# SunBangjie/FYP-BidirectionalPathTracer

Hardware: AMD Instinct MI355X
Metric: Mrays/s + RMSE vs the scalar oracle, BDPT pass, Sponza-class scene 1920x1080 depth 8 (higher is better)
Workload: dtype f32

## Files before the change

fyp-bidirectionalpathtracer_amd/__init__.py:

```python
import ctypes as C

from . import abi, tiling
from .abi import (Camera, Counters, GBuffer, GBufferParams, Params, SceneDesc, Stripes, Tile, TileInfo, load_library)

__all__ = ["abi", "tiling", "Scene", "Context", "FramePipeline", "load_library", "source_hash", "ADAPTIVE_DEFAULTS",
           "adaptive_params"]

GBUFFER_CHANNELS = ("WorldPosition", "WorldNormal", "MaterialDiffuse", "MaterialSpecRough", "MaterialExtraParams",
                    "Emissive")
OUTPUT_CHANNEL = "PipelineOutput"
AO_CHANNEL = "AmbientOcclusion"


class BdptError(RuntimeError):
    pass


def source_hash():
    import glob
    import hashlib
    import os
    here = os.path.dirname(os.path.abspath(__file__))
    root = os.path.dirname(here)
    files = sorted(glob.glob(os.path.join(here, "csrc", "*.hip")) + glob.glob(os.path.join(here, "csrc", "*.hpp")) +
# ... 856 lines not shown
        return st, fl

    def test_trace(self, rays, mode):
        import numpy as np
        rays = np.ascontiguousarray(rays, np.float32).reshape(-1, 8)
        n = rays.shape[0]
        prim = np.zeros(n, np.int32)
        tuv = np.zeros((n, 3), np.float32)
        self._check(self._lib.bdpt_test_trace(self._h, rays.ctypes.data, n, mode, prim.ctypes.data, tuv.ctypes.data),
                    "bdpt_test_trace")
        return prim, tuv

    def test_trace_shadow(self, rays):
        import numpy as np
        rays = np.ascontiguousarray(rays, np.float32)
        n = rays.shape[0]
        vis = np.zeros(n, np.uint8)
        deep = C.c_uint32(0)
        self._check(self._lib.bdpt_test_trace_shadow(self._h, rays.ctypes.data, n, vis.ctypes.data, C.byref(deep)),
                    "bdpt_test_trace_shadow")
        return vis, deep.value

    def test_bsdf(self, recs, mat_index):
        import numpy as np
        recs = np.ascontiguousarray(recs, np.float32).reshape(-1, 20)
        out = np.zeros((recs.shape[0], 16), np.float32)
        self._check(self._lib.bdpt_test_bsdf(self._h, recs.ctypes.data, recs.shape[0], mat_index, out.ctypes.data),
                    "bdpt_test_bsdf")
        return out

    def area_light_info(self):
        info = abi.AreaLightInfo()
        self._check(self._lib.bdpt_get_area_light_info(self._h, C.byref(info)), "bdpt_get_area_light_info")
        return info

    def test_area_light_sample(self, mode, states, points=None):
        import numpy as np
        states = np.ascontiguousarray(states, np.uint32).reshape(-1)
        n = states.shape[0]
        pts = None
        if points is not None:
            pts = np.ascontiguousarray(points, np.float32).reshape(n, 3)
        out = np.zeros((n, 16), np.float32)
        self._check(self._lib.bdpt_test_area_light_sample(self._h, mode, states.ctypes.data,
                                                          None if pts is None else pts.ctypes.data, n, out.ctypes.data),
                    "bdpt_test_area_light_sample")
        return out

    def test_alpha(self, variant, prim, uv):
        import numpy as np
        prim = np.ascontiguousarray(prim, np.uint32).reshape(-1)
        uv = np.ascontiguousarray(uv, np.float32).reshape(prim.shape[0], 2)
        out = np.zeros(prim.shape[0], np.uint8)
        self._check(self._lib.bdpt_test_alpha(self._h, variant, prim.ctypes.data, uv.ctypes.data, prim.shape[0], out.ctypes.data),
                    "bdpt_test_alpha")
        return out != 0

    def close(self):
        if self._h:
            self._lib.bdpt_destroy(self._h)
            self._h = None

    def __del__(self):
        try:
            self.close()
        except Exception:
# ... 348 lines not shown
```

fyp-bidirectionalpathtracer_amd/abi.py:

```python
import ctypes as C
import os

_HERE = os.path.dirname(os.path.abspath(__file__))
LIB_PATH = os.path.join(_HERE, "csrc", "libbdpt_amd.so")

BDPT_MAX_DEPTH = 16
BDPT_MAX_LIGHTS = 16
PARAM_COUNTERS = 1
PARAM_DEFER_RESOLVE = 2
PARAM_NO_NEE = 4
PARAM_NO_SPLAT = 8
PARAM_NO_CONNECT = 16
PARAM_SPECULAR_FROM_LOBE = 32
PARAM_MIS_POWER = 64
PARAM_MIS_LINEAR = 128
PARAM_DEFER_TAIL = 256
PARAM_KEEP_COUNTERS = 512
PARAM_ENV_ON_MISS = 1024
PARAM_EMISSIVE_HITS = 2048
PARAM_AREA_LIGHTS = 4096
PREPARE_PRIMARY = 1
PREPARE_BMFR = 2
PREPARE_REFIT = 4
PREPARE_LIGHT_GROUPS = 8
# ... 244 lines not shown
class WalkDesc(C.Structure):
    _fields_ = [("num", C.c_uint32), ("steps", C.c_uint32), ("numDevice", C.c_void_p), ("matIndex", C.c_uint32),
                ("flags", C.c_uint32), ("minT", C.c_float), ("reserved", C.c_uint32), ("starts", C.c_void_p), ("seeds", C.c_void_p),
                ("first", C.c_void_p), ("firstSpecular", C.c_void_p), ("alive", C.c_void_p), ("vertices", C.c_void_p),
                ("info", C.c_void_p), ("samples", C.c_void_p), ("hits", C.c_void_p)]


class AoDesc(C.Structure):
    _fields_ = [("num", C.c_uint32), ("samples", C.c_uint32), ("numDevice", C.c_void_p), ("radius", C.c_float), ("minT", C.c_float),
                ("flags", C.c_uint32), ("reserved", C.c_uint32), ("surfaces", C.c_void_p), ("seeds", C.c_void_p), ("alive", C.c_void_p),
                ("ao", C.c_void_p), ("counts", C.c_void_p), ("seedsOut", C.c_void_p)]


class AoParams(C.Structure):
    _fields_ = [("frameCount", C.c_uint32), ("radius", C.c_float), ("minT", C.c_float), ("samples", C.c_uint32),
                ("reserved", C.c_uint32)]


BMFR_MAX_PLANES = BDPT_MAX_LIGHTS + 2


class BmfrPlanesDesc(C.Structure):
    _fields_ = [("planes", C.POINTER(C.c_void_p)), ("numPlanes", C.c_uint32), ("reserved", C.c_uint32),
                ("prevPosition", C.c_void_p)]


class LightGroupDesc(C.Structure):
    _fields_ = [("planes", C.c_void_p), ("numGroups", C.c_uint32), ("numAssigned", C.c_uint32),
                ("groupOf", C.POINTER(C.c_uint8)), ("reserved", C.c_uint32 * 2)]


class AreaLightInfo(C.Structure):
    _fields_ = [("numEmitters", C.c_uint32), ("numTextured", C.c_uint32), ("totalWeight", C.c_float), ("reserved", C.c_uint32)]


PROTOTYPES = {
    "bdpt_create": (C.c_int, [C.c_int, C.POINTER(C.c_void_p)]),
    "bdpt_destroy": (None, [C.c_void_p]),
    "bdpt_last_error": (C.c_char_p, [C.c_void_p]),
    "bdpt_set_scene": (C.c_int, [C.c_void_p, C.POINTER(SceneDesc)]),
    "bdpt_get_bvh_info": (C.c_int, [C.c_void_p, C.POINTER(BvhInfo)]),
    "bdpt_set_camera": (C.c_int, [C.c_void_p, C.POINTER(Camera)]),
    "bdpt_set_environment": (C.c_int, [C.c_void_p, C.POINTER(Environment)]),
    "bdpt_bvh_build_check": (C.c_int, [C.POINTER(SceneDesc), C.POINTER(BvhInfo), C.c_char_p, C.c_uint32]),
    "bdpt_host_bvh_create": (C.c_void_p, [C.POINTER(SceneDesc), C.c_int, C.c_float, C.c_float, C.c_int, C.POINTER(BvhInfo)]),
    "bdpt_host_bvh_destroy": (None, [C.c_void_p]),
    "bdpt_host_bvh_trace": (C.c_int, [C.c_void_p, C.c_void_p, C.c_uint32, C.c_int, C.c_int, C.c_int, C.c_void_p, C.c_void_p,
                                       C.c_void_p]),
    "bdpt_update_geometry": (C.c_int, [C.c_void_p, C.POINTER(GeometryUpdate), C.c_void_p]),
    "bdpt_set_lights": (C.c_int, [C.c_void_p, C.POINTER(Light), C.c_uint32, C.c_void_p]),
    "bdpt_get_refit_info": (C.c_int, [C.c_void_p, C.POINTER(RefitInfo)]),
    "bdpt_set_skin": (C.c_int, [C.c_void_p, C.POINTER(SkinDesc)]),
    "bdpt_update_skinned": (C.c_int, [C.c_void_p, C.POINTER(SkinUpdate), C.c_void_p]),
    "bdpt_skinned_buffers": (C.c_int, [C.c_void_p, C.POINTER(C.c_void_p), C.POINTER(C.c_void_p), C.POINTER(C.c_void_p)]),
    "bdpt_host_skin": (C.c_int, [C.POINTER(SkinDesc), C.c_void_p, C.c_void_p, C.c_void_p, C.c_void_p, C.c_void_p]),
    "bdpt_test_skin_kernel": (C.c_int, [C.c_void_p, C.c_uint32, C.c_void_p]),
    "bdpt_set_morph": (C.c_int, [C.c_void_p, C.POINTER(MorphDesc)]),
    "bdpt_update_morphed": (C.c_int, [C.c_void_p, C.POINTER(MorphUpdate), C.c_void_p]),
    "bdpt_morphed_buffers": (C.c_int, [C.c_void_p, C.POINTER(C.c_void_p), C.POINTER(C.c_void_p), C.POINTER(C.c_void_p)]),
    "bdpt_host_morph": (C.c_int, [C.POINTER(MorphDesc), C.POINTER(SkinDesc), C.c_void_p, C.c_void_p, C.c_void_p, C.c_void_p, C.c_void_p,
                                  C.c_void_p]),
    "bdpt_test_morph_kernel": (C.c_int, [C.c_void_p, C.c_uint32, C.c_void_p]),
    "bdpt_trace_rays": (C.c_int, [C.c_void_p, C.POINTER(TraceDesc), C.c_void_p]),
    "bdpt_camera_rays": (C.c_int, [C.c_void_p, C.POINTER(GBufferParams), C.c_uint32, C.c_uint32, C.c_void_p, C.c_void_p]),
    "bdpt_shade_hits": (C.c_int, [C.c_void_p, C.POINTER(ShadeDesc), C.c_void_p]),
    "bdpt_bsdf_query": (C.c_int, [C.c_void_p, C.POINTER(BsdfDesc), C.c_void_p]),
# ... 33 lines not shown
    "bdpt_tile_row_ranges": (C.c_int, [C.c_void_p, C.POINTER(C.c_uint32), C.c_uint32]),
    "bdpt_resolve_tile": (C.c_int, [C.c_void_p, C.c_void_p, C.c_void_p, C.c_void_p]),
    "bdpt_accumulate_tile": (C.c_int, [C.c_void_p, C.c_void_p, C.c_void_p, C.c_uint32, C.c_uint32, C.c_void_p]),
    "bdpt_test_tree_builder": (C.c_int, [C.c_int]),
    "bdpt_bvh_recs_hash": (C.c_int, [C.POINTER(SceneDesc), C.c_int, C.POINTER(C.c_uint64), C.POINTER(BvhInfo)]),
    "bdpt_bvh_build_hash": (C.c_int, [C.POINTER(SceneDesc), C.c_int, C.POINTER(C.c_uint64), C.POINTER(BvhInfo)]),
    "bdpt_splat_buffer": (C.c_int, [C.c_void_p, C.POINTER(C.c_void_p), C.POINTER(C.c_uint64)]),
    "bdpt_set_splat_buffer": (C.c_int, [C.c_void_p, C.c_void_p, C.c_uint64]),
    "bdpt_resolve": (C.c_int, [C.c_void_p, C.c_void_p, C.c_uint32, C.c_void_p, C.c_void_p]),
    "bdpt_bmfr_execute": (C.c_int, [C.c_void_p, C.POINTER(BmfrParams), C.POINTER(GBuffer), C.c_void_p, C.c_void_p]),
    "bdpt_bmfr_execute_motion": (C.c_int, [C.c_void_p, C.POINTER(BmfrParams), C.POINTER(GBuffer), C.c_void_p, C.c_void_p, C.c_void_p]),
    "bdpt_bmfr_reset": (C.c_int, [C.c_void_p]),
    "bdpt_bmfr_history_bytes": (C.c_int, [C.c_void_p, C.POINTER(C.c_uint64)]),
    "bdpt_bmfr_save_history": (C.c_int, [C.c_void_p, C.c_void_p, C.c_uint64]),
    "bdpt_bmfr_load_history": (C.c_int, [C.c_void_p, C.c_void_p, C.c_uint64]),
    "bdpt_bmfr_execute_planes": (C.c_int, [C.c_void_p, C.POINTER(BmfrParams), C.POINTER(GBuffer), C.POINTER(BmfrPlanesDesc), C.c_void_p]),
    "bdpt_bmfr_planes_prepare": (C.c_int, [C.c_void_p, C.c_uint32]),
    "bdpt_bmfr_planes_reset": (C.c_int, [C.c_void_p]),
    "bdpt_tile_pack": (C.c_int, [C.c_void_p, C.c_void_p, C.c_void_p, C.c_uint32, C.c_void_p]),
    "bdpt_tile_unpack": (C.c_int, [C.c_void_p, C.c_uint32, C.c_void_p, C.c_void_p, C.c_uint32, C.c_void_p]),
    "bdpt_camera_view_proj": (C.c_int, [C.POINTER(C.c_float), C.POINTER(C.c_float), C.POINTER(C.c_float), C.c_float,
                                        C.c_float, C.c_float, C.c_float, C.c_float, C.POINTER(C.c_float)]),
    "bdpt_accumulate": (C.c_int, [C.c_void_p, C.c_void_p, C.c_void_p, C.c_uint32, C.c_uint32, C.c_uint64,
                                  C.c_void_p]),
    "bdpt_get_counters": (C.c_int, [C.c_void_p, C.POINTER(Counters)]),
    "bdpt_get_stage_times": (C.c_int, [C.c_void_p, C.POINTER(C.c_char_p), C.POINTER(C.c_float), C.c_int]),
    "bdpt_enable_stage_timing": (C.c_int, [C.c_void_p, C.c_int]),
    "bdpt_sync": (C.c_int, [C.c_void_p, C.c_void_p]),
    "bdpt_test_rng": (C.c_int, [C.c_void_p, C.c_void_p, C.c_void_p, C.c_uint32, C.c_uint32, C.c_void_p, C.c_void_p]),
    "bdpt_test_trace": (C.c_int, [C.c_void_p, C.c_void_p, C.c_uint32, C.c_int, C.c_void_p, C.c_void_p]),
    "bdpt_test_trace_shadow": (C.c_int, [C.c_void_p, C.c_void_p, C.c_uint32, C.c_void_p, C.c_void_p]),
    "bdpt_test_bsdf": (C.c_int, [C.c_void_p, C.c_void_p, C.c_uint32, C.c_uint32, C.c_void_p]),
    "bdpt_get_area_light_info": (C.c_int, [C.c_void_p, C.POINTER(AreaLightInfo)]),
    "bdpt_test_area_light_sample": (C.c_int, [C.c_void_p, C.c_uint32, C.c_void_p, C.c_void_p, C.c_uint32, C.c_void_p]),
    "bdpt_test_alpha": (C.c_int, [C.c_void_p, C.c_uint32, C.c_void_p, C.c_void_p, C.c_uint32, C.c_void_p]),
    "bdpt_scene_create_cornell": (C.c_void_p, []),
    "bdpt_scene_create_atrium": (C.c_void_p, [C.c_uint32, C.c_uint32]),
    "bdpt_scene_create_atrium_uneven": (C.c_void_p, [C.c_uint32, C.c_uint32]),
    "bdpt_scene_create_courtyard": (C.c_void_p, [C.c_uint32, C.c_uint32, C.c_float]),
    "bdpt_scene_create_soup": (C.c_void_p, [C.c_uint32, C.c_uint32, C.c_float]),
    "bdpt_scene_load": (C.c_void_p, [C.c_char_p, C.c_char_p, C.c_uint32]),
    "bdpt_scene_load_threads": (C.c_int, [C.c_int]),
    "bdpt_scene_destroy": (None, [C.c_void_p]),
    "bdpt_image_load": (C.c_int, [C.c_char_p, C.POINTER(C.c_uint32), C.POINTER(C.c_uint32), C.POINTER(C.c_uint32), C.c_void_p, C.c_uint64,
                                  C.c_char_p, C.c_uint32]),
    "bdpt_image_load_hdr": (C.c_int, [C.c_char_p, C.POINTER(C.c_uint32), C.POINTER(C.c_uint32), C.c_void_p, C.c_uint64, C.c_char_p, C.c_uint32]),
    "bdpt_scene_get_desc": (C.c_int, [C.c_void_p, C.POINTER(SceneDesc)]),
    "bdpt_scene_get_camera": (C.c_int, [C.c_void_p, C.c_float, C.POINTER(Camera)]),
}

_lib = None


def load_library(path=None):
    global _lib
    if _lib is not None and path is None:
        return _lib
    p = path or LIB_PATH
    if not os.path.exists(p):
        raise RuntimeError(
            f"{p} not found: the HIP extension is not built (run __graft_entry__.build()). "
            "There is no CPU fallback for the render pass.")
    lib = C.CDLL(p, mode=C.RTLD_GLOBAL)
    for name, (res, args) in PROTOTYPES.items():
        fn = getattr(lib, name)
        fn.restype = res
# ... 5 lines not shown
```

fyp-bidirectionalpathtracer_amd/csrc/api.cpp:

```cpp
#include <hip/hip_runtime.h>

#include <cmath>
#include <cstdio>
#include <cstdlib>
#include <cstring>
#include <future>
#include <functional>
#include <atomic>
#include <chrono>
#include <string>
#include <thread>
#include <vector>

#include <new>

#include "context.hpp"
#include "launch.hpp"
#include "scene_bvh.h"

using namespace bdpt;

namespace {
constexpr size_t kCountBlocks = 1;
constexpr size_t kHeadBlocks = 2;
// ... 287 lines not shown
    launchAreaRefresh(c->S, A, c->areaBlockSum, c->areaBlockLast, nullptr);
  }
  HIPCHK(c, hipGetLastError());
  HIPCHK(c, hipDeviceSynchronize());
  c->area = A;
  c->areaTextured = hc[1];
  c->areaReady = true;
  return BDPT_OK;
}

extern "C" {

int bdpt_create(int device_ordinal, bdpt_ctx** out_ctx) {
  if (!out_ctx) return BDPT_E_INVALID;
  *out_ctx = nullptr;
  int n = 0;
  if (hipGetDeviceCount(&n) != hipSuccess || n <= 0 || device_ordinal < 0 || device_ordinal >= n) return BDPT_E_HIP;
  if (hipSetDevice(device_ordinal) != hipSuccess) return BDPT_E_HIP;
  bdpt_ctx* c = new bdpt_ctx();
  c->device = device_ordinal;
  hipDeviceProp_t prop;
  if (hipGetDeviceProperties(&prop, device_ordinal) == hipSuccess && prop.multiProcessorCount > 0)
    c->numCUs = prop.multiProcessorCount;
  if (hipStreamCreateWithFlags(&c->walkStream, hipStreamNonBlocking) != hipSuccess ||
      hipEventCreateWithFlags(&c->evFork, hipEventDisableTiming) != hipSuccess ||
      hipEventCreateWithFlags(&c->evJoin, hipEventDisableTiming) != hipSuccess ||
      hipEventCreateWithFlags(&c->evSplat, hipEventDisableTiming) != hipSuccess ||
      hipEventCreateWithFlags(&c->evStage, hipEventDisableTiming) != hipSuccess ||
      hipEventCreateWithFlags(&c->evOrder, hipEventDisableTiming) != hipSuccess) {
    bdpt_destroy(c);
    return BDPT_E_HIP;
  }
  c->stackOvfStride = (uint32_t)c->numCUs * kMaxPersistentPerCU * kWave;
  if (kStackOvfRows > 0 &&
      hipMalloc(reinterpret_cast<void**>(&c->stackOvf), (size_t)kStackOvfRows * c->stackOvfStride * sizeof(int)) != hipSuccess) {
    bdpt_destroy(c);
    return BDPT_E_NOMEM;
  }
  if (hipMalloc(reinterpret_cast<void**>(&c->rayCursor), 2 * sizeof(unsigned long long)) != hipSuccess ||
      hipMemset(c->rayCursor, 0, 2 * sizeof(unsigned long long)) != hipSuccess ||
      hipMalloc(reinterpret_cast<void**>(&c->adaptiveSum), 2 * sizeof(unsigned long long)) != hipSuccess ||
      hipMemset(c->adaptiveSum, 0, 2 * sizeof(unsigned long long)) != hipSuccess) {
    bdpt_destroy(c);
    return BDPT_E_NOMEM;
  }
  bvhPrewarmStaging(device_ordinal);
  *out_ctx = c;
  return BDPT_OK;
}

void bdpt_destroy(bdpt_ctx* c) {
  if (!c) return;
  (void)hipSetDevice(c->device);
  (void)hipDeviceSynchronize();
  if (c->stackOvf) (void)hipFree(c->stackOvf);
  if (c->rayCursor) (void)hipFree(c->rayCursor);
  if (c->adaptiveSum) (void)hipFree(c->adaptiveSum);
  freeLightGroups(c);
  freeBmfrHistory(c->bmfr);
  freeBmfrHistory(c->bmfrPlanes);
  freePool(c->sceneAllocs);
  freePool(c->skinAllocs);
  freePool(c->morphAllocs);
  freePool(c->frameAllocs);
  if (c->evCreated)
    for (int i = 0; i <= kMaxStages; i++) (void)hipEventDestroy(c->ev[i]);
  if (c->evCreated)
    for (hipEvent_t e : c->sideEv) (void)hipEventDestroy(e);
  if (c->evFork) (void)hipEventDestroy(c->evFork);
  if (c->evJoin) (void)hipEventDestroy(c->evJoin);
  if (c->evSplat) (void)hipEventDestroy(c->evSplat);
// ... 2158 lines not shown
  }
  DevCounters h;
  if (e == hipSuccess) e = hipMemcpy(out_vis, dv, (size_t)n, hipMemcpyDeviceToHost);
  if (e == hipSuccess) e = hipMemcpy(&h, dcnt, sizeof(h), hipMemcpyDeviceToHost);
  freePool(pool);
  if (e != hipSuccess) {
    fail(c, hipGetErrorString(e));
    return BDPT_E_HIP;
  }
  if (out_max_stack) {
    unsigned long long m = 0;
    for (uint32_t sh = 0; sh < kCounterShards; sh++) m = std::max(m, h.v[sh][C_STACK_MAX]);
    *out_max_stack = (uint32_t)m;
  }
  return BDPT_OK;
}

int bdpt_get_area_light_info(bdpt_ctx* c, bdpt_area_light_info* out) {
  if (!c || !out) return BDPT_E_INVALID;
  if (!c->haveScene) {
    fail(c, "area_light_info: no scene (bdpt_set_scene first)");
    return BDPT_E_STATE;
  }
  ENTER(c);
  if (int rc = ensureAreaLights(c, nullptr)) return rc;
  HIPCHK(c, hipDeviceSynchronize());
  *out = bdpt_area_light_info{};
  out->numEmitters = c->area.n;
  out->numTextured = c->areaTextured;
  if (c->area.n) HIPCHK(c, hipMemcpy(&out->totalWeight, c->area.total, sizeof(float), hipMemcpyDeviceToHost));
  return BDPT_OK;
}

int bdpt_test_area_light_sample(bdpt_ctx* c, uint32_t mode, const uint32_t* states, const float* points, uint32_t n, float* out) {
  if (!c || !states || !out || mode > 1 || (mode == 1 && !points)) return BDPT_E_INVALID;
  if (!c->haveScene) {
    fail(c, "test_area_light_sample: no scene");
    return BDPT_E_STATE;
  }
  ENTER(c);
  if (int rc = ensureAreaLights(c, nullptr)) return rc;
  if (!n) return BDPT_OK;
  std::vector<void*> pool;
  const uint32_t* ds = nullptr;
  const float* dp = nullptr;
  float* dout = nullptr;
  int rc;
  if ((rc = devUpload(c, pool, &ds, states, n)) || (mode == 1 && (rc = devUpload(c, pool, &dp, points, (size_t)n * 3))) ||
      (rc = devAlloc(c, pool, &dout, (size_t)n * 16))) {
    freePool(pool);
    return rc;
  }
  hipError_t e = hipDeviceSynchronize();
  if (e == hipSuccess) {
    if (c->area.n)
      launchTestAreaSample(c->S, c->area, (int)mode, ds, dp, n, dout, nullptr);
    else
      e = hipMemset(dout, 0, (size_t)n * 64);
  }
  if (e == hipSuccess) e = hipDeviceSynchronize();
  if (e == hipSuccess) e = hipMemcpy(out, dout, (size_t)n * 64, hipMemcpyDeviceToHost);
  freePool(pool);
  if (e != hipSuccess) {
    fail(c, hipGetErrorString(e));
    return BDPT_E_HIP;
  }
// ... 60 lines not shown
```

fyp-bidirectionalpathtracer_amd/csrc/context.hpp:

```cpp
#pragma once
#include <hip/hip_runtime.h>

#include <string>
#include <utility>
#include <vector>

#include "../../include/bdpt.h"
#include "bvh.h"
#include "kernels.h"
#include "morph.h"
#include "refit.h"
#include "skin.h"

namespace bdpt {
constexpr int kMaxStages = 64;

struct BmfrHistory {
  float4* pos[2] = {nullptr, nullptr};
  float4* norm[2] = {nullptr, nullptr};
  float4 *noisy = nullptr, *filtered = nullptr;
  uint8_t* accept = nullptr;
  uint32_t* prevPixel = nullptr;
  uint32_t slots = 0;
  int read = 0;
// ... 4 lines not shown
  int device = 0;
  int numCUs = 256;
  std::string err;
  bool haveScene = false, haveCamera = false, haveSize = false;
  bdpt::SceneDev S{};
  std::vector<void*> sceneAllocs;
  bdpt_bvh_info bvhInfo{};
  bdpt_camera cam{};
  bdpt_environment env{};
  uint32_t W = 0, H = 0, maxDepth = 0;
  std::vector<std::pair<uint32_t, uint32_t>> rowRanges;
  uint32_t tileRows = 0;
  bdpt::SplatLayout sl{1, 1, 0};
  bdpt_stripes stripes{0, 1, 0};
  bdpt::PathBuf P{};
  std::vector<void*> frameAllocs;
  unsigned long long* splat = nullptr;
  unsigned long long* ownSplat = nullptr;
  bdpt::DevCounters* counters = nullptr;
  hipStream_t lastStream = nullptr;
  bool timing = false;
  hipEvent_t ev[bdpt::kMaxStages + 1]{};
  const char* stageNames[bdpt::kMaxStages]{};
  int numStages = 0;
  bool evCreated = false;
  static constexpr int kMaxSideStages = 4;
  hipEvent_t sideEv[2 * kMaxSideStages]{};
  const char* sideNames[kMaxSideStages]{};
  int numSideStages = 0;
  int lazyRounds = 3;
  bdpt::LaunchGrids grids{};
  int* stackOvf = nullptr;
  uint32_t stackOvfStride = 0;
  unsigned long long* rayCursor = nullptr;
  unsigned long long* adaptiveSum = nullptr;
  bdpt_gbuffer ownGb{};
  bdpt::BmfrHistory bmfr, bmfrPlanes;
  hipStream_t walkStream = nullptr;
  hipEvent_t evFork = nullptr, evJoin = nullptr, evSplat = nullptr;
  uint32_t* hintPix = nullptr;
  bool hints = true;
  bdpt_camera hintCam{};
  bool hintCamValid = false;
  uint32_t numVertices = 0, numTriangles = 0;
  uint32_t* lightMaps = nullptr;
  bool refitReady = false;
  bdpt::BvhRefitPlan refitPlan;
  bdpt::RefitDev refit{};
  uint32_t numUpdates = 0;
  float* stage[3] = {nullptr, nullptr, nullptr};
  void* pinned = nullptr;
  size_t pinnedBytes = 0;
  hipEvent_t evStage = nullptr, evOrder = nullptr;
  bool stageInFlight = false;
  unsigned long long* groupSplat = nullptr;
  uint32_t groupSplatPlanes = 0;
  uint8_t* groupLightIdx = nullptr;
  const uint32_t* alphaTris = nullptr;
  uint32_t numAlphaTris = 0;
  bool areaReady = false;
  bdpt::AreaDev area{};
  uint32_t areaTextured = 0;
  float* areaBlockSum = nullptr;
  uint32_t* areaBlockLast = nullptr;
  std::vector<void*> skinAllocs;
  bool haveSkin = false;
// ... 33 lines not shown
```

fyp-bidirectionalpathtracer_amd/csrc/device_trace.hpp:

```cpp
#pragma once
#include "bvh.h"
#include "device_scene.hpp"

namespace bdpt {
#define BD __device__ __forceinline__
#define BDPT_ONE_WAVE_PER_GROUP()               \
  do {                                          \
    if (blockDim.x != (unsigned)kWave) return;  \
  } while (0)

struct Hit {
  int prim;
  float t, u, v;
  uint32_t rec;
};

constexpr int kDone = (int)0x80000000;

struct TravState {
  f3 o, d, idir;
  uint32_t neg;
  float tmin, tmax;
  int cur, sp;
  Hit best;
};

BD float clampedRcp(float d) {
  float r = 1.0f / d;
  if (!(fabsf(r) <= 1.0e30f)) r = copysignf(1.0e30f, d);
  return r;
}

BD void travInit(TravState& T, f3 o, f3 d, float tmin, float tmax) {
  T.o = o;
  T.d = d;
  T.idir = mk(clampedRcp(d.x), clampedRcp(d.y), clampedRcp(d.z));
  T.neg = (__float_as_uint(d.x) >> 31) | ((__float_as_uint(d.y) >> 31) << 1) | ((__float_as_uint(d.z) >> 31) << 2);
  T.tmin = tmin;
  T.tmax = tmax;
  T.sp = 0;
  T.best.prim = -1;
  T.best.t = tmax;
  T.best.u = 0.0f;
  T.best.v = 0.0f;
  T.best.rec = 0xFFFFFFFFu;
  const bool finite = (o.x == o.x) && (o.y == o.y) && (o.z == o.z) && (d.x == d.x) && (d.y == d.y) && (d.z == d.z);
  T.cur = (finite && (tmax > tmin)) ? 0 : kDone;
}

template <int KL>
BD int* ovfSlot(const SceneDev& S, int e) {
  return S.stackOvf + (size_t)(e - KL) * S.stackOvfStride + (size_t)blockIdx.x * kWave + (threadIdx.x & 63u);
}
template <int KL>
BD void stackStore(const SceneDev& S, int* stk, int e, int ref) {
  if (KL < kStackEntries && e >= KL)
    *ovfSlot<KL>(S, e) = ref;
  else
    stk[e * kWave] = ref;
}
template <int KL>
BD int travPop(const SceneDev& S, TravState& T, const int* stk) {
  if (T.sp == 0) return kDone;
  T.sp--;
  if (KL < kStackEntries && T.sp >= KL) return *ovfSlot<KL>(S, T.sp);
  return stk[T.sp * kWave];
}
template <int KL>
BD void travPush(const SceneDev& S, TravState& T, int* stk, int ref) {
  stackStore<KL>(S, stk, T.sp, ref);
  T.sp++;
}

BD float ubyte(uint32_t w, int c) { return (float)((w >> (8 * c)) & 0xffu); }

template <int ORDER, int KL = kStackEntries>
BD void nodeStep(const SceneDev& S, TravState& T, int* stk) {
  const uint4* np = S.recs + (size_t)T.cur * kRecF4;
  const uint4 q0 = np[0], q1 = np[1], q2 = np[2];
  const float sx = __uint_as_float((q0.w << 23) & 0x7f800000u), sy = __uint_as_float((q0.w << 15) & 0x7f800000u),
              sz = __uint_as_float((q0.w << 7) & 0x7f800000u);
  const float ax = sx * T.idir.x, ay = sy * T.idir.y, az = sz * T.idir.z;
  const float bx = (__uint_as_float(q0.x) - T.o.x) * T.idir.x, by = (__uint_as_float(q0.y) - T.o.y) * T.idir.y,
              bz = (__uint_as_float(q0.z) - T.o.z) * T.idir.z;
  const bool nx = (T.neg & 1u) != 0, ny = (T.neg & 2u) != 0, nz = (T.neg & 4u) != 0;
  const uint32_t nearX = nx ? q1.w : q1.x, farX = nx ? q1.x : q1.w;
  const uint32_t nearY = ny ? q2.x : q1.y, farY = ny ? q1.y : q2.x;
  const uint32_t nearZ = nz ? q2.y : q1.z, farZ = nz ? q1.z : q2.y;
  float tn[4];
  bool hit[4];
#pragma unroll
  for (int c = 0; c < 4; c++) {
    const float tnx = fmaf(ubyte(nearX, c), ax, bx), tfx = fmaf(ubyte(farX, c), ax, bx);
    const float tny = fmaf(ubyte(nearY, c), ay, by), tfy = fmaf(ubyte(farY, c), ay, by);
    const float tnz = fmaf(ubyte(nearZ, c), az, bz), tfz = fmaf(ubyte(farZ, c), az, bz);
    const float n = fmaxf(fmaxf(tnx, tny), fmaxf(tnz, T.tmin));
    const float f = fminf(fminf(tfx, tfy), fminf(tfz, T.best.t));
    hit[c] = n <= f;
    tn[c] = n;
  }
  int r0 = (int)q2.z ^ ((int)(q0.w << 7) >> 31);
  int r1 = (int)(q2.z + ((q2.w >> 8) & 0xffu)) ^ ((int)(q0.w << 6) >> 31);
  int r2 = (int)(q2.z + ((q2.w >> 16) & 0xffu)) ^ ((int)(q0.w << 5) >> 31);
  int r3 = (int)(q2.z + (q2.w >> 24)) ^ ((int)(q0.w << 4) >> 31);
// ... 415 lines not shown
```

fyp-bidirectionalpathtracer_amd/csrc/kernels.h:

```cpp
#pragma once
#include <hip/hip_runtime.h>
#include <stdint.h>

#include "../../include/bdpt.h"
#include "texture_planes.h"

namespace bdpt {

constexpr int kWave = 64;
#ifndef KSTACK
#define KSTACK 32
#endif
constexpr int kStackEntries = KSTACK;
#ifndef BDPT_STACK_LDS
#define BDPT_STACK_LDS 24
#endif
constexpr int kStackLds = BDPT_STACK_LDS < KSTACK ? BDPT_STACK_LDS : KSTACK;
#ifndef BDPT_WALK_STACK_LDS
#define BDPT_WALK_STACK_LDS 28
#endif
constexpr int kWalkStackLds = BDPT_WALK_STACK_LDS < KSTACK ? BDPT_WALK_STACK_LDS : KSTACK;
constexpr int kMaxPersistentPerCU = 32;
constexpr int kStackOvfRows = KSTACK - (kStackLds < kWalkStackLds ? kStackLds : kWalkStackLds);
constexpr int kShadeRecF4 = 8;
constexpr uint32_t kNoRay = 0xFFFFFFFFu;
constexpr uint32_t kNumSubQueues = 32;
#ifndef BDPT_FETCH_CHUNK
#define BDPT_FETCH_CHUNK 256
#endif
constexpr uint32_t kFetchChunk = BDPT_FETCH_CHUNK;
constexpr uint32_t kCursorStride = 32;
constexpr uint32_t kCursorBlock = kNumSubQueues * kCursorStride;
#ifndef BDPT_RAY_SUBQUEUES
#define BDPT_RAY_SUBQUEUES 32
#endif
constexpr uint32_t kNumRaySubQueues = BDPT_RAY_SUBQUEUES;
constexpr uint32_t kRayCursorBlock = kNumRaySubQueues * kCursorStride;
constexpr uint32_t kCounterShards = 64;

enum : int { F_COL = 0, F_POS = 3, F_N = 6, F_V = 9, F_DIF = 12, F_SPEC = 15, F_ROUGH = 18, F_ISSPEC = 19, F_PDF = 20, NF = 21 };
constexpr int NF4 = 6;
enum : int { PATH_EYE = 0, PATH_LIGHT = 1 };
enum : int { RAY_TERMS = 0, RAY_PAIRS = 1 };

struct TexDev {
  const uint8_t* px;
  uint32_t w, h, srgb, pow2;
};

struct SceneConst {
  bdpt_light lights[BDPT_MAX_LIGHTS];
  float srgbLut[256];
};

struct SceneDev {
  const uint4* recs;
// ... 312 lines not shown
```

fyp-bidirectionalpathtracer_amd/csrc/kernels.hip:

```cpp
#include "kernels.h"

#include <algorithm>
#include <type_traits>

#include "device_area.hpp"
#include "device_connect.hpp"
#include "device_math.hpp"
#include "device_motion.hpp"
#include "device_scene.hpp"
#include "device_trace.hpp"
#include "launch.hpp"

namespace bdpt {

#define BD __device__ __forceinline__

BD void wavePush(bool active, uint32_t value, uint32_t* items, uint32_t* count, uint32_t subCap, uint32_t q = 0xffffffffu) {
  unsigned long long mask = __ballot(active);
  if (mask == 0ull) return;
  const int lane = (int)(threadIdx.x & 63u);
  const int leader = __ffsll((long long)mask) - 1;
  if (q == 0xffffffffu) q = blockIdx.x % kNumSubQueues;
  uint32_t base = 0;
  if (lane == leader) base = atomicAdd(&count[q * kCursorStride], (uint32_t)__popcll(mask));
// ... 284 lines not shown
  wavePush(geom, p, P.queue[0], P.qcount, P.pathSubCap);
  if (MASKED) wavePush(geom && active, p, M.eye, M.eyeCount, P.pathSubCap);
}
template <bool GGX, FrameKind V>
__global__ __launch_bounds__(kWave) void init_paths_kernel(SceneDev S, FrameDev F, PathBuf P, FrameArg<V> A) {
  BDPT_ONE_WAVE_PER_GROUP();
  initPathsLane<GGX, V == FrameKind::Groups, V == FrameKind::Masked>(S, F, P, groupOf(A), maskOf(A));
}
template <bool GGX, FrameKind V>
__global__ __launch_bounds__(kWave) void init_paths_area_kernel(SceneDev S, FrameDev F, PathBuf P, FrameArg<V> A, AreaDev E) {
  BDPT_ONE_WAVE_PER_GROUP();
  initPathsLane<GGX, V == FrameKind::Groups, V == FrameKind::Masked, true>(S, F, P, groupOf(A), maskOf(A), E);
}

constexpr uint32_t kPoolEntries = 128;
#ifndef BDPT_WALK_ORDER
#define BDPT_WALK_ORDER 1
#endif
#ifndef BDPT_WALK_SHADE_MIN
#define BDPT_WALK_SHADE_MIN 64
#endif
#ifndef BDPT_WALK_LEAF_WAIT
#define BDPT_WALK_LEAF_WAIT 1
#endif
#ifndef BDPT_WALK_NODE_BURST
#define BDPT_WALK_NODE_BURST 3
#endif
#ifndef BDPT_WALK_CHUNK
#define BDPT_WALK_CHUNK 64
#endif
#ifndef BDPT_WALK_REFILL
#define BDPT_WALK_REFILL BDPT_REFILL_IDLE
#endif
BD uint32_t packPath(uint32_t p, int path, int k) { return p | ((uint32_t)path << 24) | ((uint32_t)k << 25); }

#ifndef BDPT_WALK_WAVES_PER_EU
#define BDPT_WALK_WAVES_PER_EU 4
#endif
constexpr uint32_t kParkedMiss = 1u << 30;
template <bool GGX, bool COUNT, bool EXT, bool MASKED>
__global__ __launch_bounds__(kWave) __attribute__((amdgpu_waves_per_eu(BDPT_WALK_WAVES_PER_EU, 8))) void walk_kernel(
    SceneDev S, FrameDev F, PathBuf P, uint32_t* __restrict__ head, FrameArg<MASKED ? FrameKind::Masked : FrameKind::Plain> mask) {
  BDPT_ONE_WAVE_PER_GROUP();
  __shared__ int s_stack[kWalkStackLds * kWave];
  __shared__ uint4 s_pool[kPoolEntries];
  __shared__ float s_srgb[256];
#pragma unroll
  for (int i = 0; i < 256; i += kWave) s_srgb[i + (int)threadIdx.x] = S.sc->srgbLut[i + (int)threadIdx.x];
  __syncthreads();
  ldsF32* const srgb = (ldsF32*)s_srgb;
  const MaskDev& M = maskOf(mask);
  int* stk = s_stack + threadIdx.x;
  const int lane = (int)(threadIdx.x & 63u);
  const unsigned long long laneBelow = (1ull << lane) - 1ull;
  const int D = (int)F.p.maxDepth;
  const bool fromLobe = (F.p.flags & BDPT_PARAM_SPECULAR_FROM_LOBE) != 0;
  const uint32_t firstV = (D >= 2) ? 0u : kNumSubQueues, numV = 2u * kNumSubQueues - firstV;
  bool trav = false;
  uint32_t id = 0;
  TravState T;
  travInit(T, mk(0), mk(0), F.p.minT, 1.0e38f);
  T.cur = kDone;
  uint32_t nNodes = 0, nTris = 0, nAlpha = 0;
  uint32_t nEye = 0, nLight = 0, nParked = 0, nReady = 0;
  uint32_t vq = firstV + blockIdx.x % numV, tried = 0, chunkPos = 0, chunkEnd = 0, chunk = BDPT_WALK_CHUNK;
  bool exhausted = false;
  const uint32_t wavesPerList = (gridDim.x + numV - 1) / numV;
  for (;;) {
    unsigned long long travMask = __ballot(trav);
    const bool flush = (travMask == 0ull) && nReady == 0 && exhausted && nParked > 0;
    if (nParked >= (uint32_t)BDPT_WALK_SHADE_MIN || flush) {
      const uint32_t n = nParked < (uint32_t)kWave ? nParked : (uint32_t)kWave;
      nParked -= n;
      const bool act = (uint32_t)lane < n;
      uint4 rec = make_uint4(0, 0, 0, 0);
      if (act) rec = s_pool[nParked + (uint32_t)lane];
      __syncthreads();
      const uint32_t p = rec.x & 0xffffffu;
      const int path = (int)((rec.x >> 24) & 1u), k = (int)((rec.x >> 25) & 31u);
      nEye += (uint32_t)__popcll(__ballot(act && path == PATH_EYE));
      nLight += (uint32_t)__popcll(__ballot(act && path == PATH_LIGHT));
      bool survive = false;
      f3 L = mk(0);
      if (act) {
        const bool miss = EXT ? (rec.x & kParkedMiss) != 0u : (int)rec.y < 0;
        const int prim = miss ? -1 : (int)rec.y;
        const float4* rk = vtxPtr(P, path, k, p);
        const float4 qc = rk[0], qp = rk[1];
        const f3 o = mk(qp.x, qp.y, qp.z);
        f3 found = mk(0);
        bool haveFound = false;
        if (prim >= 0) {
          const uint32_t seed = __float_as_uint(qc.w);
          const f3 thr = mk(qc.x, qc.y, qc.z);
          Shading sd = shadeHitLut<false>(S, srgb, (uint32_t)prim, __uint_as_float(rec.z), __uint_as_float(rec.w), o);
          float pdf;
          bool isSpec;
          f3 w = sampleBRDF<GGX>(seed, sd.N, sd.N, sd.V, sd.diffuse, sd.specular, sd.roughness, fromLobe, L, pdf, isSpec);
          Vtx v;
          v.color = thr * w;
          v.pos = sd.posW;
          v.N = sd.N;
          v.V = sd.V;
          v.dif = sd.diffuse;
          v.spec = sd.specular;
          v.rough = sd.roughness;
          v.isSpec = isSpec;
          v.pdf = pdf;
          v.seed = seed;
          storeVtx(P, path, k + 1, p, v);
// ... 13 lines not shown
          Vtx g = zeroVtx();
          if (path == PATH_EYE && k == 1) {
            g.pos = o;
          } else {
            loadSurf(P, path, k, p, g);
            g.V = ldPlane3(P, path, k, F_V, p);
            if (path == PATH_LIGHT && k == 0) g.pdf = 0.0f;
          }
          g.color = mk(0);
          storeVtx(P, path, k + 1, p, g);
          if (path == PATH_EYE) {
            P.eyeLast[p] = (uint8_t)(k + 1);
          } else {
            P.lightLast[p] = (uint8_t)(k + 1);
            P.lightReal[p] = (uint8_t)k;
          }
        }
        if (MASKED && haveFound && M.mask[P.pix[p]] == 0) haveFound = false;
        if (EXT && haveFound) {
          f3 term = clampVec(found / (float)(k + 1), F.p.clampUpper);
          if (isnan3(term)) term = mk(0);
          float4* out4 = reinterpret_cast<float4*>(F.out);
          const size_t pix = P.pix[p];
          float4 acc = out4[pix];
          acc.x = acc.x + term.x;
          acc.y = acc.y + term.y;
          acc.z = acc.z + term.z;
          acc.w = acc.w + 1.0f;
          out4[pix] = acc;
        }
      }
      const unsigned long long sm = __ballot(survive);
      if (survive) {
        const uint32_t slot = kPoolEntries - 1u - nReady - (uint32_t)__popcll(sm & laneBelow);
        s_pool[slot] = make_uint4(packPath(p, path, k + 1), __float_as_uint(L.x), __float_as_uint(L.y), __float_as_uint(L.z));
      }
      nReady += (uint32_t)__popcll(sm);
      __builtin_amdgcn_fence(__ATOMIC_RELEASE, "workgroup");
      __syncthreads();
    }
    const int empty = 64 - __popcll(travMask);
    if ((empty >= BDPT_WALK_REFILL || travMask == 0ull) && (nReady > 0 || !exhausted)) {
      const unsigned long long emptyMask = ~travMask;
      const uint32_t rank = (uint32_t)__popcll(emptyMask & laneBelow);
      const uint32_t fromReady = ((uint32_t)empty < nReady) ? (uint32_t)empty : nReady;
      bool got = false;
      uint32_t nid = 0;
      f3 dir = mk(0);
      if (!trav && rank < fromReady) {
        const uint4 r = s_pool[kPoolEntries - nReady + rank];
        nid = r.x;
        dir = mk(__uint_as_float(r.y), __uint_as_float(r.z), __uint_as_float(r.w));
        got = true;
      }
      __syncthreads();
      nReady -= fromReady;
      uint32_t want = (uint32_t)empty - fromReady;
      uint32_t taken = fromReady;
      while (want > 0 && !exhausted) {
        while (chunkPos >= chunkEnd && !exhausted) {
          const uint32_t* counts = (MASKED && vq < kNumSubQueues) ? M.walkEyeCount : P.qcount;
          const uint32_t nq = counts[(vq % kNumSubQueues) * kCursorStride];
          uint32_t base = nq;
          if (__hip_atomic_load(&head[vq * kCursorStride], __ATOMIC_RELAXED, __HIP_MEMORY_SCOPE_AGENT) < nq) {
            uint32_t share = (nq / wavesPerList + 15u) & ~15u;
            chunk = share < 16u ? 16u : (share > (uint32_t)BDPT_WALK_CHUNK ? (uint32_t)BDPT_WALK_CHUNK : share);
            if (lane == 0) base = atomicAdd(&head[vq * kCursorStride], chunk);
            base = (uint32_t)__builtin_amdgcn_readfirstlane((int)base);
          }
          if (base < nq) {
            chunkPos = base;
            chunkEnd = (base + chunk < nq) ? base + chunk : nq;
            tried = 0;
          } else {
            vq = (vq + 1 == 2u * kNumSubQueues) ? firstV : vq + 1;
            if (++tried >= numV) exhausted = true;
          }
// ... 37 lines not shown
      if ((int)__popcll(waitMask) >= waitNeed || nodeMask == 0ull) {
        if (trav && T.cur < 0) {
          finished = (T.cur == kDone);
          if (!finished) {
            finished = leafStep<0, COUNT>(S, T, nTris, nAlpha);
            if (!finished) {
              T.cur = travPop<kWalkStackLds>(S, T, stk);
              finished = (T.cur == kDone);
            }
          }
        }
      }
    }
#else
    if (trav) {
      while (T.cur >= 0) {
        if (COUNT) nNodes++;
        nodeStep<BDPT_WALK_ORDER, kWalkStackLds>(S, T, stk);
      }
      finished = (T.cur == kDone);
      if (!finished) {
        finished = leafStep<0, COUNT>(S, T, nTris, nAlpha);
        if (!finished) {
          T.cur = travPop<kWalkStackLds>(S, T, stk);
          finished = (T.cur == kDone);
        }
      }
    }
#endif
    const unsigned long long finMask = __ballot(finished);
    if (finMask) {
      if (finished) {
        const bool miss = T.best.prim < 0;
        s_pool[nParked + (uint32_t)__popcll(finMask & laneBelow)] =
            (EXT && miss) ? make_uint4(id | kParkedMiss, __float_as_uint(T.d.x), __float_as_uint(T.d.y), __float_as_uint(T.d.z))
                          : make_uint4(id, (uint32_t)T.best.prim, __float_as_uint(T.best.u), __float_as_uint(T.best.v));
        trav = false;
      }
      nParked += (uint32_t)__popcll(finMask);
      __syncthreads();
    }
  }
  if (lane == 0) {
    if (nEye) atomicAdd(&F.counters->v[blockIdx.x % kCounterShards][C_RAYS_EYE], (unsigned long long)nEye);
    if (nLight) atomicAdd(&F.counters->v[blockIdx.x % kCounterShards][C_RAYS_LIGHT], (unsigned long long)nLight);
  }
  if (COUNT) {
    waveAddCount(F.counters, C_NODE_CLOSEST, nNodes);
    waveAddCount(F.counters, C_TRI_CLOSEST, nTris);
    waveAddCount(F.counters, C_ALPHA_CLOSEST, nAlpha);
  }
}

BD float evalGWithoutVPos(f3 posA, f3 nA, f3 posB, f3 nB) {
  const f3 vecAB = posB - posA;
  const float invLengthAB = 1.0f / length(vecAB);
  const f3 dirAB = vecAB * invLengthAB;
  const float cosA = fabsf(dot(nA, dirAB));
  const float cosB = fabsf(dot(nB, dirAB));
  return cosA * cosB * invLengthAB * invLengthAB;
}

__global__ __launch_bounds__(kWave) void mis_prefix_kernel(FrameDev F, PathBuf P) {
  BDPT_ONE_WAVE_PER_GROUP();
  bool act = false;
  uint32_t i = 0;
  if (!queueChunk(P.qcount, P.pathSubCap, act, i)) return;
// ... 1083 lines not shown
```

include/bdpt.h:

```cpp
#ifndef BDPT_H_
#define BDPT_H_

#include <stdint.h>

#ifdef __cplusplus
extern "C" {
#endif

#define BDPT_OK 0
#define BDPT_E_INVALID (-1)
#define BDPT_E_STATE (-2)
#define BDPT_E_HIP (-3)
#define BDPT_E_NOMEM (-4)
#define BDPT_E_LIMIT (-5)

#define BDPT_MAX_LIGHTS 16
#define BDPT_MAX_DEPTH 16

#define BDPT_LIGHT_POINT 0
#define BDPT_LIGHT_DIRECTIONAL 1

#define BDPT_SHADING_MODEL_METAL_ROUGH 0u
#define BDPT_SHADING_MODEL_SPEC_GLOSS 2u
#define BDPT_CHANNEL_UNUSED 0u
// ... 615 lines not shown
#define BDPT_BMFR_MAX_PLANES (BDPT_MAX_LIGHTS + 2)
typedef struct bdpt_bmfr_planes_desc {
  float* const* planes;
  uint32_t numPlanes;
  uint32_t reserved;
  const float* prevPosition;
} bdpt_bmfr_planes_desc;
int bdpt_bmfr_execute_planes(bdpt_ctx* ctx, const bdpt_bmfr_params* p, const bdpt_gbuffer* features,
                             const bdpt_bmfr_planes_desc* desc, void* stream);
int bdpt_bmfr_planes_prepare(bdpt_ctx* ctx, uint32_t numPlanes);
int bdpt_bmfr_planes_reset(bdpt_ctx* ctx);

int bdpt_tile_pack(bdpt_ctx* ctx, const void* frame, void* packed, uint32_t bytesPerPixel, void* stream);
int bdpt_tile_unpack(bdpt_ctx* ctx, uint32_t owner, const void* packed, void* frame, uint32_t bytesPerPixel, void* stream);

int bdpt_camera_view_proj(const float pos[3], const float target[3], const float up[3], float focalLengthMm,
                          float frameHeightMm, float aspect, float nearZ, float farZ, float out16[16]);

int bdpt_get_counters(bdpt_ctx* ctx, bdpt_counters* out);

int bdpt_get_stage_times(bdpt_ctx* ctx, const char** names, float* ms, int cap);
int bdpt_enable_stage_timing(bdpt_ctx* ctx, int enable);

int bdpt_sync(bdpt_ctx* ctx, void* stream);

typedef struct bdpt_area_light_info {
  uint32_t numEmitters;
  uint32_t numTextured;
  float totalWeight;
  uint32_t reserved;
} bdpt_area_light_info;
int bdpt_get_area_light_info(bdpt_ctx* ctx, bdpt_area_light_info* out);

int bdpt_test_rng(bdpt_ctx* ctx, const uint32_t* val0, const uint32_t* val1, uint32_t n, uint32_t draws,
                  uint32_t* out_states, float* out_floats);
int bdpt_test_trace(bdpt_ctx* ctx, const float* rays, uint32_t n, int mode, int32_t* out_prim, float* out_tuv);
int bdpt_test_trace_shadow(bdpt_ctx* ctx, const float* rays, uint32_t n, uint8_t* out_vis, uint32_t* out_max_stack);
int bdpt_test_bsdf(bdpt_ctx* ctx, const float* in, uint32_t n, uint32_t matIndex, float* out);
int bdpt_test_area_light_sample(bdpt_ctx* ctx, uint32_t mode, const uint32_t* states, const float* points, uint32_t n, float* out);
int bdpt_test_alpha(bdpt_ctx* ctx, uint32_t variant, const uint32_t* prim, const float* uv, uint32_t n, uint8_t* out_fails);
int bdpt_test_skin_kernel(bdpt_ctx* ctx, uint32_t path, void* stream);
int bdpt_test_morph_kernel(bdpt_ctx* ctx, uint32_t path, void* stream);

#ifdef __cplusplus
}
#endif
#endif
```

Measured before the change: 4989.

## Stash traversal state across walk shading phase to cut registers and raise occupancy

```diff
diff --git a/fyp-bidirectionalpathtracer_amd/__init__.py b/fyp-bidirectionalpathtracer_amd/__init__.py
--- a/fyp-bidirectionalpathtracer_amd/__init__.py
+++ b/fyp-bidirectionalpathtracer_amd/__init__.py
@@ -912,6 +912,11 @@
     def area_light_info(self):
         info = abi.AreaLightInfo()
         self._check(self._lib.bdpt_get_area_light_info(self._h, C.byref(info)), "bdpt_get_area_light_info")
+        return info
+
+    def stack_info(self):
+        info = abi.StackInfo()
+        self._check(self._lib.bdpt_get_stack_info(self._h, C.byref(info)), "bdpt_get_stack_info")
         return info
 
     def test_area_light_sample(self, mode, states, points=None):
diff --git a/fyp-bidirectionalpathtracer_amd/abi.py b/fyp-bidirectionalpathtracer_amd/abi.py
--- a/fyp-bidirectionalpathtracer_amd/abi.py
+++ b/fyp-bidirectionalpathtracer_amd/abi.py
@@ -300,6 +300,11 @@
 
 class AreaLightInfo(C.Structure):
     _fields_ = [("numEmitters", C.c_uint32), ("numTextured", C.c_uint32), ("totalWeight", C.c_float), ("reserved", C.c_uint32)]
+
+
+class StackInfo(C.Structure):
+    _fields_ = [("entries", C.c_uint32), ("ldsRows", C.c_uint32), ("walkLdsRows", C.c_uint32), ("walkStashRows", C.c_uint32),
+                ("overflowStride", C.c_uint32), ("reserved", C.c_uint32), ("overflowWords", C.c_uint64)]
 
 
 PROTOTYPES = {
@@ -399,6 +404,7 @@
     "bdpt_test_trace_shadow": (C.c_int, [C.c_void_p, C.c_void_p, C.c_uint32, C.c_void_p, C.c_void_p]),
     "bdpt_test_bsdf": (C.c_int, [C.c_void_p, C.c_void_p, C.c_uint32, C.c_uint32, C.c_void_p]),
     "bdpt_get_area_light_info": (C.c_int, [C.c_void_p, C.POINTER(AreaLightInfo)]),
+    "bdpt_get_stack_info": (C.c_int, [C.c_void_p, C.POINTER(StackInfo)]),
     "bdpt_test_area_light_sample": (C.c_int, [C.c_void_p, C.c_uint32, C.c_void_p, C.c_void_p, C.c_uint32, C.c_void_p]),
     "bdpt_test_alpha": (C.c_int, [C.c_void_p, C.c_uint32, C.c_void_p, C.c_void_p, C.c_uint32, C.c_void_p]),
     "bdpt_scene_create_cornell": (C.c_void_p, []),
diff --git a/fyp-bidirectionalpathtracer_amd/csrc/api.cpp b/fyp-bidirectionalpathtracer_amd/csrc/api.cpp
--- a/fyp-bidirectionalpathtracer_amd/csrc/api.cpp
+++ b/fyp-bidirectionalpathtracer_amd/csrc/api.cpp
@@ -343,11 +343,16 @@
     return BDPT_E_HIP;
   }
   c->stackOvfStride = (uint32_t)c->numCUs * kMaxPersistentPerCU * kWave;
+  if ((uint64_t)kStackOvfRows * c->stackOvfStride >= (1ull << 30)) {
+    bdpt_destroy(c);
+    return BDPT_E_NOMEM;
+  }
   if (kStackOvfRows > 0 &&
       hipMalloc(reinterpret_cast<void**>(&c->stackOvf), (size_t)kStackOvfRows * c->stackOvfStride * sizeof(int)) != hipSuccess) {
     bdpt_destroy(c);
     return BDPT_E_NOMEM;
   }
+  c->stackOvfWords = c->stackOvf ? (uint64_t)kStackOvfRows * c->stackOvfStride : 0;
   if (hipMalloc(reinterpret_cast<void**>(&c->rayCursor), 2 * sizeof(unsigned long long)) != hipSuccess ||
       hipMemset(c->rayCursor, 0, 2 * sizeof(unsigned long long)) != hipSuccess ||
       hipMalloc(reinterpret_cast<void**>(&c->adaptiveSum), 2 * sizeof(unsigned long long)) != hipSuccess ||
@@ -2572,6 +2577,18 @@
   return BDPT_OK;
 }
 
+int bdpt_get_stack_info(const bdpt_ctx* c, bdpt_stack_info* out) {
+  if (!c || !out) return BDPT_E_INVALID;
+  *out = bdpt_stack_info{};
+  out->entries = (uint32_t)kStackEntries;
+  out->ldsRows = (uint32_t)kStackLds;
+  out->walkLdsRows = (uint32_t)kWalkStackLds;
+  out->walkStashRows = (uint32_t)kWalkStashRows;
+  out->overflowStride = c->stackOvfStride;
+  out->overflowWords = c->stackOvfWords;
+  return BDPT_OK;
+}
+
 int bdpt_test_area_light_sample(bdpt_ctx* c, uint32_t mode, const uint32_t* states, const float* points, uint32_t n, float* out) {
   if (!c || !states || !out || mode > 1 || (mode == 1 && !points)) return BDPT_E_INVALID;
   if (!c->haveScene) {
diff --git a/fyp-bidirectionalpathtracer_amd/csrc/context.hpp b/fyp-bidirectionalpathtracer_amd/csrc/context.hpp
--- a/fyp-bidirectionalpathtracer_amd/csrc/context.hpp
+++ b/fyp-bidirectionalpathtracer_amd/csrc/context.hpp
@@ -60,6 +60,7 @@
   bdpt::LaunchGrids grids{};
   int* stackOvf = nullptr;
   uint32_t stackOvfStride = 0;
+  uint64_t stackOvfWords = 0;
   unsigned long long* rayCursor = nullptr;
   unsigned long long* adaptiveSum = nullptr;
   bdpt_gbuffer ownGb{};
diff --git a/fyp-bidirectionalpathtracer_amd/csrc/device_trace.hpp b/fyp-bidirectionalpathtracer_amd/csrc/device_trace.hpp
--- a/fyp-bidirectionalpathtracer_amd/csrc/device_trace.hpp
+++ b/fyp-bidirectionalpathtracer_amd/csrc/device_trace.hpp
@@ -50,7 +50,8 @@
 
 template <int KL>
 BD int* ovfSlot(const SceneDev& S, int e) {
-  return S.stackOvf + (size_t)(e - KL) * S.stackOvfStride + (size_t)blockIdx.x * kWave + (threadIdx.x & 63u);
+  const uint32_t w = (uint32_t)(e - KL) * S.stackOvfStride + blockIdx.x * (uint32_t)kWave + (threadIdx.x & 63u);
+  return S.stackOvf + w;
 }
 template <int KL>
 BD void stackStore(const SceneDev& S, int* stk, int e, int ref) {
@@ -70,6 +71,41 @@
 BD void travPush(const SceneDev& S, TravState& T, int* stk, int ref) {
   stackStore<KL>(S, stk, T.sp, ref);
   T.sp++;
+}
+
+template <int KL>
+BD void travStash(const SceneDev& S, const TravState& T, int* stk) {
+  static_assert(KL < kStackEntries, "entries past the LDS rows need the overflow area");
+  const float w[kTravStashRows] = {T.o.x, T.o.y, T.o.z, T.d.x, T.d.y, T.d.z, T.best.t, T.best.u, T.best.v};
+  if (T.sp <= KL - kTravStashRows) {
+    int* c = stk + T.sp * kWave;
+#pragma unroll
+    for (int i = 0; i < kTravStashRows; i++) c[i * kWave] = (int)__float_as_uint(w[i]);
+  } else {
+    int* g = ovfSlot<KL>(S, T.sp > KL ? T.sp : KL);
+#pragma unroll
+    for (int i = 0; i < kTravStashRows; i++) g[(uint32_t)i * S.stackOvfStride] = (int)__float_as_uint(w[i]);
+  }
+}
+template <int KL>
+BD void travUnstash(const SceneDev& S, TravState& T, const int* stk) {
+  float w[kTravStashRows];
+  if (T.sp <= KL - kTravStashRows) {
+    const int* c = stk + T.sp * kWave;
+#pragma unroll
+    for (int i = 0; i < kTravStashRows; i++) w[i] = __uint_as_float((uint32_t)c[i * kWave]);
+  } else {
+    const int* g = ovfSlot<KL>(S, T.sp > KL ? T.sp : KL);
+#pragma unroll
+    for (int i = 0; i < kTravStashRows; i++) w[i] = __uint_as_float((uint32_t)g[(uint32_t)i * S.stackOvfStride]);
+  }
+  T.o = mk(w[0], w[1], w[2]);
+  T.d = mk(w[3], w[4], w[5]);
+  T.idir = mk(clampedRcp(T.d.x), clampedRcp(T.d.y), clampedRcp(T.d.z));
+  T.neg = (__float_as_uint(T.d.x) >> 31) | ((__float_as_uint(T.d.y) >> 31) << 1) | ((__float_as_uint(T.d.z) >> 31) << 2);
+  T.best.t = w[6];
+  T.best.u = w[7];
+  T.best.v = w[8];
 }
 
 BD float ubyte(uint32_t w, int c) { return (float)((w >> (8 * c)) & 0xffu); }
diff --git a/fyp-bidirectionalpathtracer_amd/csrc/kernels.h b/fyp-bidirectionalpathtracer_amd/csrc/kernels.h
--- a/fyp-bidirectionalpathtracer_amd/csrc/kernels.h
+++ b/fyp-bidirectionalpathtracer_amd/csrc/kernels.h
@@ -17,11 +17,17 @@
 #endif
 constexpr int kStackLds = BDPT_STACK_LDS < KSTACK ? BDPT_STACK_LDS : KSTACK;
 #ifndef BDPT_WALK_STACK_LDS
-#define BDPT_WALK_STACK_LDS 28
+#define BDPT_WALK_STACK_LDS 20
 #endif
 constexpr int kWalkStackLds = BDPT_WALK_STACK_LDS < KSTACK ? BDPT_WALK_STACK_LDS : KSTACK;
+#ifndef BDPT_WALK_STASH
+#define BDPT_WALK_STASH 1
+#endif
+constexpr int kTravStashRows = 9;
+constexpr int kWalkStashRows = BDPT_WALK_STASH ? kTravStashRows : 0;
 constexpr int kMaxPersistentPerCU = 32;
-constexpr int kStackOvfRows = KSTACK - (kStackLds < kWalkStackLds ? kStackLds : kWalkStackLds);
+constexpr int kWalkOvfRows = kWalkStackLds < KSTACK ? KSTACK - kWalkStackLds + kWalkStashRows : 0;
+constexpr int kStackOvfRows = (KSTACK - kStackLds) > kWalkOvfRows ? (KSTACK - kStackLds) : kWalkOvfRows;
 constexpr int kShadeRecF4 = 8;
 constexpr uint32_t kNoRay = 0xFFFFFFFFu;
 constexpr uint32_t kNumSubQueues = 32;
diff --git a/fyp-bidirectionalpathtracer_amd/csrc/kernels.hip b/fyp-bidirectionalpathtracer_amd/csrc/kernels.hip
--- a/fyp-bidirectionalpathtracer_amd/csrc/kernels.hip
+++ b/fyp-bidirectionalpathtracer_amd/csrc/kernels.hip
@@ -340,14 +340,19 @@
 #ifndef BDPT_WALK_REFILL
 #define BDPT_WALK_REFILL BDPT_REFILL_IDLE
 #endif
+BD int lanesBelow(unsigned long long mask) {
+  return (int)__builtin_amdgcn_mbcnt_hi((uint32_t)(mask >> 32), __builtin_amdgcn_mbcnt_lo((uint32_t)mask, 0u));
+}
 BD uint32_t packPath(uint32_t p, int path, int k) { return p | ((uint32_t)path << 24) | ((uint32_t)k << 25); }
 
 #ifndef BDPT_WALK_WAVES_PER_EU
-#define BDPT_WALK_WAVES_PER_EU 4
+#define BDPT_WALK_WAVES_PER_EU 5
 #endif
+constexpr int walkWavesPerEu(bool count, bool ext) { return (count || ext) ? 4 : BDPT_WALK_WAVES_PER_EU; }
 constexpr uint32_t kParkedMiss = 1u << 30;
+static_assert(BDPT_WALK_SHADE_MIN <= kWave, "the pool bound, and with it the free entries the stash uses, needs fewer than 64 records parked at a fetch");
 template <bool GGX, bool COUNT, bool EXT, bool MASKED>
-__global__ __launch_bounds__(kWave) __attribute__((amdgpu_waves_per_eu(BDPT_WALK_WAVES_PER_EU, 8))) void walk_kernel(
+__global__ __launch_bounds__(kWave) __attribute__((amdgpu_waves_per_eu(walkWavesPerEu(COUNT, EXT), 8))) void walk_kernel(
     SceneDev S, FrameDev F, PathBuf P, uint32_t* __restrict__ head, FrameArg<MASKED ? FrameKind::Masked : FrameKind::Plain> mask) {
   BDPT_ONE_WAVE_PER_GROUP();
   __shared__ int s_stack[kWalkStackLds * kWave];
@@ -360,7 +365,6 @@
   const MaskDev& M = maskOf(mask);
   int* stk = s_stack + threadIdx.x;
   const int lane = (int)(threadIdx.x & 63u);
-  const unsigned long long laneBelow = (1ull << lane) - 1ull;
   const int D = (int)F.p.maxDepth;
   const bool fromLobe = (F.p.flags & BDPT_PARAM_SPECULAR_FROM_LOBE) != 0;
   const uint32_t firstV = (D >= 2) ? 0u : kNumSubQueues, numV = 2u * kNumSubQueues - firstV;
@@ -383,7 +387,14 @@
       const bool act = (uint32_t)lane < n;
       uint4 rec = make_uint4(0, 0, 0, 0);
       if (act) rec = s_pool[nParked + (uint32_t)lane];
+#if BDPT_WALK_STASH
+      const uint32_t stashSlot = nParked + (uint32_t)lanesBelow(travMask);
+      if (trav) travStash<kWalkStackLds>(S, T, stk);
+#endif
       __syncthreads();
+#if BDPT_WALK_STASH
+      if (trav) s_pool[stashSlot] = make_uint4((uint32_t)T.sp, id, (uint32_t)T.cur, (uint32_t)T.best.prim);
+#endif
       const uint32_t p = rec.x & 0xffffffu;
       const int path = (int)((rec.x >> 24) & 1u), k = (int)((rec.x >> 25) & 31u);
       nEye += (uint32_t)__popcll(__ballot(act && path == PATH_EYE));
@@ -463,17 +474,29 @@
       }
       const unsigned long long sm = __ballot(survive);
       if (survive) {
-        const uint32_t slot = kPoolEntries - 1u - nReady - (uint32_t)__popcll(sm & laneBelow);
+        const uint32_t slot = kPoolEntries - 1u - nReady - (uint32_t)lanesBelow(sm);
         s_pool[slot] = make_uint4(packPath(p, path, k + 1), __float_as_uint(L.x), __float_as_uint(L.y), __float_as_uint(L.z));
       }
       nReady += (uint32_t)__popcll(sm);
       __builtin_amdgcn_fence(__ATOMIC_RELEASE, "workgroup");
       __syncthreads();
+#if BDPT_WALK_STASH
+      {
+        const uint4 st = s_pool[stashSlot];
+        T.sp = trav ? (int)st.x : 0;
+        id = st.y;
+        T.cur = trav ? (int)st.z : kDone;
+        T.best.prim = (int)st.w;
+        T.tmin = F.p.minT;
+        T.tmax = 1.0e38f;
+        travUnstash<kWalkStackLds>(S, T, stk);
+      }
+#endif
     }
     const int empty = 64 - __popcll(travMask);
     if ((empty >= BDPT_WALK_REFILL || travMask == 0ull) && (nReady > 0 || !exhausted)) {
       const unsigned long long emptyMask = ~travMask;
-      const uint32_t rank = (uint32_t)__popcll(emptyMask & laneBelow);
+      const uint32_t rank = (uint32_t)lanesBelow(emptyMask);
       const uint32_t fromReady = ((uint32_t)empty < nReady) ? (uint32_t)empty : nReady;
       bool got = false;
       uint32_t nid = 0;
@@ -577,7 +600,7 @@
     if (finMask) {
       if (finished) {
         const bool miss = T.best.prim < 0;
-        s_pool[nParked + (uint32_t)__popcll(finMask & laneBelow)] =
+        s_pool[nParked + (uint32_t)lanesBelow(finMask)] =
             (EXT && miss) ? make_uint4(id | kParkedMiss, __float_as_uint(T.d.x), __float_as_uint(T.d.y), __float_as_uint(T.d.z))
                           : make_uint4(id, (uint32_t)T.best.prim, __float_as_uint(T.best.u), __float_as_uint(T.best.v));
         trav = false;
diff --git a/include/bdpt.h b/include/bdpt.h
--- a/include/bdpt.h
+++ b/include/bdpt.h
@@ -671,6 +671,13 @@
 } bdpt_area_light_info;
 int bdpt_get_area_light_info(bdpt_ctx* ctx, bdpt_area_light_info* out);
 
+typedef struct bdpt_stack_info {
+  uint32_t entries, ldsRows, walkLdsRows, walkStashRows;
+  uint32_t overflowStride, reserved;
+  uint64_t overflowWords;
+} bdpt_stack_info;
+int bdpt_get_stack_info(const bdpt_ctx* ctx, bdpt_stack_info* out);
+
 int bdpt_test_rng(bdpt_ctx* ctx, const uint32_t* val0, const uint32_t* val1, uint32_t n, uint32_t draws,
                   uint32_t* out_states, float* out_floats);
 int bdpt_test_trace(bdpt_ctx* ctx, const float* rays, uint32_t n, int mode, int32_t* out_prim, float* out_tuv);
```

New measurement: 5028 (median of 6 runs). Within noise of the previous version (+0.8%).
